# pairlab/SlotFormer

Measured on AMD Instinct MI355X. Metric: rollout frames/sec at B=32, 128x128, 7 slots, 6+50 steps (SAVi-encode + SlotFormer rollout), higher is better.
Workload: dtype f32 storage; matmul/conv on split-bf16 MFMA (bf16x3: hi*hi+hi*lo+lo*hi, f32 accumulate)

## Files before the change

slotformer_amd/csrc/layer_tok.hip:

```cpp
#include "../../include/slotformer_hip.h"
#include "sf_internal.h"
#include "layer_fused.h"
#include "layer_tok_common.h"
#include <stdlib.h>

namespace {
constexpr int LT_NT = 256, LT_D = 256, LT_F = 1024, LT_NH = 8, LT_TOK = 128, LT_MAXL = 8;
constexpr int LT_STAGE = 32 * 1024, LT_RING = 3;
constexpr int LT_NST_ATT = 4 * LT_NH, LT_NST = LT_NST_ATT + 2 * (LT_F / 32);
constexpr int LT_KV = LT_RING * LT_STAGE;
constexpr int LT_VT = LT_KV + 16 * 1024;
constexpr int LT_PAR = LT_KV + 32 * 1024;
constexpr int P_LN1G = 0, P_LN1B = 256, P_BQKV = 512, P_BO = 1280, P_LN2G = 1536, P_LN2B = 1792, P_B1 = 2048, P_B2 = 3072, P_N = 3328;
constexpr size_t LT_LDS = (size_t)LT_PAR + (size_t)P_N * 4;
constexpr size_t LT_BLOB = (size_t)LT_NST * LT_STAGE + (size_t)P_N * 4;
static_assert(LT_LDS <= 160 * 1024, "LDS budget");

struct LtArgs {
  const float* x;
  const float* ring;
  const float* pe;
  float* y;
  const char* blob[LT_MAXL];
  float eps;
  int nl, B, L, vpw, RF, N, f0, dbg_ts;
};
}

__device__ long long lt_ts[16];
#define LTS(i) do { if (A.dbg_ts && blockIdx.x == 0 && threadIdx.x == 0) lt_ts[i] = wall_clock64(); } while (0)

template <int MODE>
__global__ __launch_bounds__(LT_NT) void layer_tok_kernel(LtArgs A) {
  extern __shared__ __attribute__((aligned(16))) char smem[];
  float* P = (float*)(smem + LT_PAR);
  const int t = threadIdx.x, lane = t & 63;
  const int wave = __builtin_amdgcn_readfirstlane(t >> 6);
  const int n = lane & 31, h = lane >> 5;
  const int L = A.L;
  const int v0 = blockIdx.x * A.vpw;
  const int nvalid = min(A.vpw, A.B - v0) * L;
  const int tl = wave * 32 + n;
  const int te = min(tl, nvalid - 1);
  const int vl = te / L, tok = te - vl * L;
  const long long row = (long long)(v0 + vl) * L + tok;
  LTS(0);
  f32x16 X[8];
  if constexpr (MODE == 0) {
    const float* xr = A.x + row * LT_D + 4 * h;
#pragma unroll
    for (int ob = 0; ob < 8; ++ob)
#pragma unroll
      for (int g = 0; g < 4; ++g) {
        const f32x4 v = *(const f32x4*)(xr + 32 * ob + 8 * g);
#pragma unroll
        for (int q = 0; q < 4; ++q) X[ob][4 * g + q] = v[q];
      }
  } else {
    const int fr = tok / A.N, sl = tok - fr * A.N;
    const float* rr = A.ring + (((long long)(v0 + vl) * A.RF + (A.f0 + fr) % A.RF) * A.N + sl) * LT_D + 4 * h;
    const float* pr = A.pe + (long long)tok * LT_D + 4 * h;
#pragma unroll
    for (int ob = 0; ob < 8; ++ob)
#pragma unroll
      for (int g = 0; g < 4; ++g) {
        const f32x4 v = *(const f32x4*)(rr + 32 * ob + 8 * g);
#pragma unroll
        for (int q = 0; q < 4; ++q) X[ob][4 * g + q] = v[q];
      }
    __builtin_amdgcn_sched_barrier(0);
#pragma unroll
    for (int ob = 0; ob < 8; ++ob) {
#pragma unroll
      for (int g = 0; g < 4; ++g) {
        const f32x4 v = *(const f32x4*)(pr + 32 * ob + 8 * g);
#pragma unroll
        for (int q = 0; q < 4; ++q) X[ob][4 * g + q] += v[q];
      }
      __builtin_amdgcn_sched_barrier(0);
    }
  }
  const unsigned wlane = (unsigned)(wave * 8 * 1024 + lane * 16);
  char* const wdst = smem + (wave * 8) * 1024;
  int cur = 0;
  int cs = -2;
  const char* base_cur = A.blob[0];
  const char* base_nxt = A.blob[0];
  bool last_layer = false;
  auto stage_src = [&]() -> const char* {
    const int t2 = cs + 2;
    const bool wrap = t2 >= LT_NST;
    const char* b = wrap ? base_nxt : base_cur;
    const int so = wrap ? (last_layer ? LT_NST - 1 : t2 - LT_NST) : t2;
    ++cs;
    return b + (size_t)so * LT_STAGE + wlane;
  };
  {
    const char* s0 = stage_src();
    const char* s1 = stage_src();
    LtRing R0{nullptr, s0, wdst}, R1{nullptr, s1, wdst + LT_STAGE};
#pragma unroll
    for (int f = 0; f < 8; ++f) lt_dma(R0, f);
#pragma unroll
    for (int f = 0; f < 8; ++f) lt_dma(R1, f);
  }
#ifdef LT_STAMPS
  long long c_wait = 0, c_bar = 0, c_last = 0, c_work = 0;
#endif
  auto stage_begin = [&]() -> LtRing {
#ifdef LT_STAMPS
    const long long c0 = __builtin_readcyclecounter();
    if (c_last) c_work += c0 - c_last;
#endif
#ifdef LT_NODMA
    asm volatile("s_waitcnt vmcnt(0)" ::: "memory");
#else
    asm volatile("s_waitcnt vmcnt(8)" ::: "memory");
#endif
    asm volatile("s_waitcnt lgkmcnt(0)" ::: "memory");
#ifdef LT_STAMPS
    const long long c1 = __builtin_readcyclecounter();
#endif
#ifndef LT_NOBAR
    __builtin_amdgcn_s_barrier();
#endif
    asm volatile("" ::: "memory");
#ifdef LT_STAMPS
    c_last = __builtin_readcyclecounter();
    c_wait += c1 - c0;
    c_bar += c_last - c1;
#endif
    const int nb = cur == 0 ? 2 : cur - 1;
    LtRing R{smem + cur * LT_STAGE + lane * 16, stage_src(), wdst + nb * LT_STAGE};
#ifdef LT_BURST
#pragma unroll
    for (int f = 0; f < 8; ++f) lt_dma_now(R, f);
#endif
    cur = cur == 2 ? 0 : cur + 1;
    return R;
  };
  const int wf = min(wave * 32, nvalid - 1);
  const int kb0 = ((wf / L) * L) >> 5;
  const int d0 = 32 * kb0 + 4 * h - vl * L;
  const char* pb;
  {
    unsigned pbo = (unsigned)(LT_PAR + 16 * h);
    asm volatile("" : "+v"(pbo));
    pb = smem + pbo;
  }
  char* const kwr = smem + LT_KV + wave * 1024 + lane * 16;
  char* const vwr = smem + LT_VT + wave * 4096 + lane * 16;
  const char* krd[3];
  const char* vrd[3];
#pragma unroll
  for (int kbi = 0; kbi < 3; ++kbi) {
    const int kb = min(kb0 + kbi, 3);
    krd[kbi] = smem + LT_KV + kb * 1024 + lane * 16;
    vrd[kbi] = smem + LT_VT + kb * 4096 + lane * 16;
  }
  const float qscale = 0.2550348616841918f;
  constexpr float NEG = -3.0e38f;
  LTS(1);

#pragma unroll 1
  for (int l = 0; l < A.nl; ++l) {
    cs = 0;
    base_cur = A.blob[l];
    last_layer = l + 1 >= A.nl;
    base_nxt = A.blob[last_layer ? l : l + 1];
    __syncthreads();
    {
      const float* vsrc = (const float*)(A.blob[l] + (size_t)LT_NST * LT_STAGE);
      for (int i = t; i < P_N / 4; i += LT_NT) *(f32x4*)(P + 4 * i) = *(const f32x4*)(vsrc + 4 * i);
    }
    __syncthreads();
    if (l == 0) LTS(2);
    bf16x8 xh[16], xl[16];
    lt_layernorm<P_LN1G, P_LN1B>(X, pb, h, A.eps, xh, xl);
    lt_add_vec<P_BO>(X, pb);
    if (l == 0) LTS(3);
    f32x16 qa, ka, va, S[3], O;
    bf16x8 qh[2], ql[2], ph[3][2], pl[3][2], oh[2], ol[2];
    float mx0 = NEG, mx1 = NEG, mx = 0.f, sm = 0.f, rinv = 0.f;
    auto zero16 = [](f32x16& a) {
#pragma unroll
      for (int r = 0; r < 16; ++r) a[r] = 0.f;
    };
    int hq = 0;
    auto mask_chunk = [&](int c) {
      const int kbi = c >> 1;
#pragma unroll
      for (int rr = 0; rr < 8; ++rr) {
        const int r = 8 * (c & 1) + rr;
        const bool ok = (unsigned)(d0 + 32 * kbi + 8 * (r >> 2) + (r & 3)) < (unsigned)L;
        const float v = ok ? S[kbi][r] : NEG;
        S[kbi][r] = v;
        if (rr & 1) mx1 = fmaxf(mx1, v); else mx0 = fmaxf(mx0, v);
      }
    };
    auto exp_chunk = [&](int c) {
      const int kbi = c >> 1;
      float s0 = 0.f, s1 = 0.f;
#pragma unroll
      for (int rr = 0; rr < 8; ++rr) {
        const int r = 8 * (c & 1) + rr;
#ifdef LT_EXPF
        const float e = __expf((S[kbi][r] - mx) * 0.6931471805599453f);
#else
        const float e = __builtin_amdgcn_exp2f(S[kbi][r] - mx);
#endif
        S[kbi][r] = e;
        if (rr & 1) s1 += e; else s0 += e;
      }
      sm += s0 + s1;
    };
    auto psplit_chunk = [&](int c) { split8(quad(S[c >> 1], 2 * (c & 1)), quad(S[c >> 1], 2 * (c & 1) + 1), ph[c >> 1][c & 1], pl[c >> 1][c & 1]); };
    auto kconv = [&](int s) {
      const float* bk = (const float*)pb + P_BQKV + 256 + 32 * hq;
      bf16x8 fh, fl;
      split8(quad(ka, 2 * s) + *(const f32x4*)(bk + 16 * s), quad(ka, 2 * s + 1) + *(const f32x4*)(bk + 16 * s + 8), fh, fl);
      *(bf16x8*)(kwr + (s * 2) * 4096) = fh;
      *(bf16x8*)(kwr + (s * 2 + 1) * 4096) = fl;
    };
    auto qconv = [&](int s) {
      const float* bq = (const float*)pb + P_BQKV + 32 * hq;
      split8((quad(qa, 2 * s) + *(const f32x4*)(bq + 16 * s)) * qscale, (quad(qa, 2 * s + 1) + *(const f32x4*)(bq + 16 * s + 8)) * qscale, qh[s], ql[s]);
    };
    auto vconv = [&](int s) {
      const float bv = P[P_BQKV + 512 + 32 * hq + n];
      bf16x8 fh, fl;
      split8(quad(va, 2 * s) + bv, quad(va, 2 * s + 1) + bv, fh, fl);
      *(bf16x8*)(vwr + (s * 2) * 1024) = fh;
      *(bf16x8*)(vwr + (s * 2 + 1) * 1024) = fl;
    };
    auto oconv = [&](int s) { split8(quad(O, 2 * s) * rinv, quad(O, 2 * s + 1) * rinv, oh[s], ol[s]); };
    auto scores = [&]() {
      bf16x8 kh[3][2], kl[3][2];
#pragma unroll
      for (int kbi = 0; kbi < 3; ++kbi)
#pragma unroll
        for (int s = 0; s < 2; ++s) {
          kh[kbi][s] = *(const bf16x8*)(krd[kbi] + (s * 2) * 4096);
          kl[kbi][s] = *(const bf16x8*)(krd[kbi] + (s * 2 + 1) * 4096);
        }
#pragma unroll
      for (int kbi = 0; kbi < 3; ++kbi) zero16(S[kbi]);
#pragma unroll
      for (int s = 0; s < 2; ++s) {
#pragma unroll
        for (int kbi = 0; kbi < 3; ++kbi) { S[kbi] = LT_MFMA(kh[kbi][s], ql[s], S[kbi]); LT_PIN(); }
#pragma unroll
        for (int kbi = 0; kbi < 3; ++kbi) { S[kbi] = LT_MFMA(kl[kbi][s], qh[s], S[kbi]); LT_PIN(); }
#pragma unroll
        for (int kbi = 0; kbi < 3; ++kbi) { S[kbi] = LT_MFMA(kh[kbi][s], qh[s], S[kbi]); LT_PIN(); }
      }
      mx0 = mx1 = NEG;
      sm = 0.f;
    };
    auto pv = [&]() {
      f32x16 Op[3];
      bf16x8 vh[3][2], vlo[3][2];
#pragma unroll
      for (int kbi = 0; kbi < 3; ++kbi)
#pragma unroll
        for (int s = 0; s < 2; ++s) {
          vh[kbi][s] = *(const bf16x8*)(vrd[kbi] + (s * 2) * 1024);
          vlo[kbi][s] = *(const bf16x8*)(vrd[kbi] + (s * 2 + 1) * 1024);
        }
#pragma unroll
      for (int kbi = 0; kbi < 3; ++kbi) zero16(Op[kbi]);
#pragma unroll
      for (int s = 0; s < 2; ++s) {
#pragma unroll
        for (int kbi = 0; kbi < 3; ++kbi) { Op[kbi] = LT_MFMA(vh[kbi][s], pl[kbi][s], Op[kbi]); LT_PIN(); }
#pragma unroll
        for (int kbi = 0; kbi < 3; ++kbi) { Op[kbi] = LT_MFMA(vlo[kbi][s], ph[kbi][s], Op[kbi]); LT_PIN(); }
#pragma unroll
        for (int kbi = 0; kbi < 3; ++kbi) { Op[kbi] = LT_MFMA(vh[kbi][s], ph[kbi][s], Op[kbi]); LT_PIN(); }
      }
#pragma unroll
      for (int r = 0; r < 16; ++r) O[r] = (Op[0][r] + Op[1][r]) + Op[2][r];
    };
    auto sideD = [&](int g) {
      if (g < 6) mask_chunk(g);
      if (g == 6) mx = lt_xmax(fmaxf(mx0, mx1), h);
      if (g == 7) exp_chunk(0);
    };
    auto sideA = [&](int g) {
      if (g == 0) { exp_chunk(1); exp_chunk(2); }
      if (g == 1) { exp_chunk(3); exp_chunk(4); }
      if (g == 2) { exp_chunk(5); rinv = 1.0f / lt_xsum(sm, h); psplit_chunk(0); }
      if (g == 3) { psplit_chunk(1); psplit_chunk(2); }
      if (g == 4) { psplit_chunk(3); psplit_chunk(4); }
      if (g == 5) psplit_chunk(5);
    };
    {
      const LtRing R = stage_begin();
      lt_row_product<false, 0>(R, xh, xl, qa, LtNoSide{});
    }
    {
      const LtRing R = stage_begin();
      lt_row_product<false, 0>(R, xh, xl, ka, LtNoSide{});
    }
    {
      const LtRing R = stage_begin();
      lt_row_product<true, 5>(R, xh, xl, va, [&](int g) {
        if (g < 2) kconv(g);
        else if (g < 4) qconv(g - 2);
      });
      vconv(0);
      vconv(1);
    }
#pragma unroll 1
    for (hq = 1; hq < LT_NH; ++hq) {
      {
        const LtRing R = stage_begin();
        scores();
          lt_row_product<false, 6>(R, xh, xl, qa, sideD);
      }
      {
        const LtRing R = stage_begin();
          lt_row_product<false, 6>(R, xh, xl, ka, sideA);
        pv();
      }
      {
        const LtRing R = stage_begin();
          lt_row_product<true, 5>(R, xh, xl, va, [&](int g) {
          if (g < 2) kconv(g);
          else if (g < 4) qconv(g - 2);
          else if (g < 6) oconv(g - 4);
        });
      }
      {
        const LtRing R = stage_begin();
        lt_kslice_product<5>(R, oh, ol, X, [&](int g) {
          if (g < 2) vconv(g);
        });
      }
    }
    asm volatile("s_waitcnt lgkmcnt(0)" ::: "memory");
    __builtin_amdgcn_s_barrier();
    asm volatile("" ::: "memory");
    scores();
#pragma unroll
    for (int g = 0; g < 8; ++g) sideD(g);
#pragma unroll
    for (int g = 0; g < 6; ++g) sideA(g);
    pv();
    oconv(0);
    oconv(1);
    {
      const LtRing R = stage_begin();
      lt_kslice_product<0>(R, oh, ol, X, LtNoSide{});
    }
    if (l == 0) LTS(4);
#ifdef LT_STAMPS
    if (l == 0 && blockIdx.x == 0 && threadIdx.x == 0) { lt_ts[8] = c_wait; lt_ts[9] = c_bar; lt_ts[10] = c_work; }
#endif
    lt_layernorm<P_LN2G, P_LN2B>(X, pb, h, A.eps, xh, xl);
    lt_add_vec<P_B2>(X, pb);
    if (l == 0) LTS(5);
    f32x16 Ha, Hb;
    bf16x8 hh[2], hl[2];
    f32x4 b1q[4];
    auto b1_load = [&](int blk) {
      const float* b1 = (const float*)pb + P_B1 + 32 * blk;
#pragma unroll
      for (int g = 0; g < 4; ++g) b1q[g] = *(const f32x4*)(b1 + 8 * g);
    };
    auto hconv = [&](const f32x16& Hx, int s) {
      const f32x4 z4 = {0.f, 0.f, 0.f, 0.f};
      const f32x4 u0 = __builtin_elementwise_max(quad(Hx, 2 * s) + b1q[2 * s], z4);
      const f32x4 u1 = __builtin_elementwise_max(quad(Hx, 2 * s + 1) + b1q[2 * s + 1], z4);
      split8(u0, u1, hh[s], hl[s]);
    };
    auto ffn_step = [&](f32x16& Hn, const f32x16& Hp, int j) {
      {
        const LtRing R = stage_begin();
        lt_row_product<false, 4>(R, xh, xl, Hn, [&](int g) {
          if (g >= 1 && g < 3) hconv(Hp, g - 1);
        });
        asm volatile("" : "+v"(hh[0]), "+v"(hh[1]), "+v"(hl[0]), "+v"(hl[1]));
      }
      {
        const LtRing R = stage_begin();
        b1_load(j);
        lt_kslice_product<0>(R, hh, hl, X, LtNoSide{});
      }
    };
    {
      const LtRing R = stage_begin();
      b1_load(0);
      lt_row_product<false, 0>(R, xh, xl, Ha, LtNoSide{});
    }
    ffn_step(Hb, Ha, 1);
#pragma unroll 1
    for (int j = 2; j < LT_F / 32; j += 2) {
      ffn_step(Ha, Hb, j);
      ffn_step(Hb, Ha, j + 1);
    }
    hconv(Hb, 0);
    hconv(Hb, 1);
    {
      const LtRing R = stage_begin();
      lt_kslice_product<0>(R, hh, hl, X, LtNoSide{});
    }
    if (l == 0) LTS(6);
#ifdef LT_STAMPS
    if (l == 0 && blockIdx.x == 0 && threadIdx.x == 0) { lt_ts[11] = c_wait; lt_ts[12] = c_bar; lt_ts[13] = c_work; }
#endif
  }
  asm volatile("s_waitcnt vmcnt(0)" ::: "memory");
  if (tl < nvalid) {
    float* yr = A.y + row * LT_D + 4 * h;
#pragma unroll
    for (int ob = 0; ob < 8; ++ob)
#pragma unroll
      for (int g = 0; g < 4; ++g) *(f32x4*)(yr + 32 * ob + 8 * g) = quad(X[ob], g);
  }
  LTS(7);
}

extern "C" int sf_debug_read_ts_layer_tok(long long* out16) {
  hipError_t e = hipMemcpyFromSymbol(out16, HIP_SYMBOL(lt_ts), sizeof(long long) * 16);
  return e == hipSuccess ? 0 : (int)e;
}

extern "C" size_t sf_layer_tok_packed_bytes(void) { return LT_BLOB; }
extern "C" size_t sf_layer_tok_packed_bytes_ex(int d_model, int num_heads, int ffn) {
  if (d_model == LT_D && num_heads == LT_NH && ffn == LT_F) return LT_BLOB;
  return sf_layer_tok128_shape(d_model, num_heads, ffn) ? sf_layer_tok128_packed_bytes() : 0;
}

extern "C" int sf_pack_layer_tok_weights(const sf_tfm_layer* w, void* packed, int d_model, int num_heads, int ffn, void* stream) {
  SF_REQUIRE(w && packed, "sf_pack_layer_tok_weights: null pointer");
  SF_REQUIRE(w->in_proj_w && w->out_proj_w && w->lin1_w && w->lin2_w && w->norm1_g && w->norm1_b && w->in_proj_b && w->out_proj_b && w->norm2_g &&
                 w->norm2_b && w->lin1_b && w->lin2_b, "sf_pack_layer_tok_weights: null weight");
  hipStream_t st = (hipStream_t)stream;
  if (sf_layer_tok128_shape(d_model, num_heads, ffn)) return sf_pack_layer_tok128(w, packed, st);
  SF_REQUIRE(d_model == LT_D && num_heads == LT_NH && ffn == LT_F, "sf_pack_layer_tok_weights: (d_model, heads, ffn) = (256, 8, 1024) or (128, 8, 512) only");
  const int total = LT_NST * 32 * 64;
  hipLaunchKernelGGL((pack_layer_tok_kernel<LT_D, LT_F>), dim3((total + 255) / 256), dim3(256), 0, st, w->in_proj_w, w->out_proj_w, w->lin1_w, w->lin2_w, (uint4*)packed);
  SF_CHECK_LAUNCH();
  float* vec = (float*)((char*)packed + (size_t)LT_NST * LT_STAGE);
  const struct {
    const float* src;
    int off, n;
  } parts[8] = {{w->norm1_g, P_LN1G, 256}, {w->norm1_b, P_LN1B, 256}, {w->in_proj_b, P_BQKV, 768}, {w->out_proj_b, P_BO, 256},
                {w->norm2_g, P_LN2G, 256}, {w->norm2_b, P_LN2B, 256}, {w->lin1_b, P_B1, 1024},   {w->lin2_b, P_B2, 256}};
  for (const auto& p : parts) {
    const hipError_t e = hipMemcpyAsync(vec + p.off, p.src, (size_t)p.n * 4, hipMemcpyDeviceToDevice, st);
    if (e != hipSuccess) return sf_set_err((int)e, hipGetErrorString(e), __FILE__, __LINE__);
  }
  return 0;
}

int sf_layer_tok_vpw(int L) {
  if (L < 1 || L > 96) return 0;
  for (int vpw = LT_TOK / L; vpw >= 1; --vpw) {
    const int nvalid = vpw * L;
    bool ok = true;
    for (int w = 0; w < 4 && ok; ++w) {
      const int wf = w * 32 < nvalid ? w * 32 : nvalid - 1, wl = w * 32 + 31 < nvalid ? w * 32 + 31 : nvalid - 1;
      const int kb0 = ((wf / L) * L) >> 5, kb1 = (((wl / L) * L) + L - 1) >> 5;
      ok = kb1 - kb0 + 1 <= 3;
    }
    if (ok) return vpw;
  }
  return 0;
}
bool sf_layer_tok_ok(int L) { return sf_layer_tok_vpw(L) > 0; }

int sf_layer_tok_ex(int mode, const float* xin, const float* ring, int ring_frames, int nslots, int f0, const float* pe, const sf_tfm_layer* layers, int nl,
                    float eps, float* y, int B, int L, hipStream_t st) {
  bool ok = layers && nl >= 1 && nl <= LT_MAXL && sf_layer_tok_ok(L) && B >= 1 && y && (mode == 0 ? xin != nullptr : (ring && pe && nslots >= 1 && ring_frames >= 1));
  for (int l = 0; ok && l < nl; ++l) ok = layers[l].tok_packed != nullptr;
  if (!ok)
    return sf_set_err(-1, "invalid argument: the token-stationary layers need sf_pack_layer_tok_weights fragments, 1..8 layers and 1 <= L <= 96 rows per video", __FILE__, __LINE__);
  static const int dbg = sf_dbg("lt");
  LtArgs A;
  A.x = xin; A.ring = ring; A.pe = pe; A.y = y;
  for (int l = 0; l < LT_MAXL; ++l) A.blob[l] = (const char*)layers[l < nl ? l : nl - 1].tok_packed;
  A.eps = eps; A.nl = nl; A.B = B; A.L = L; A.vpw = sf_layer_tok_vpw(L); A.RF = ring_frames; A.N = nslots; A.f0 = f0; A.dbg_ts = dbg;
  const int nwg = (B + A.vpw - 1) / A.vpw;
  const double flops = nl * ((double)B * L * (2.0 * LT_D * (3 * LT_D + LT_D + 2 * LT_F)) + (double)B * LT_NH * 4.0 * L * L * 32);
  if (mode == 0) {
    SF_TRY(sf_ensure_dyn_lds((const void*)layer_tok_kernel<0>, LT_LDS));
    sf_prof_begin(SF_K_LAYER_TOK, st, flops);
    hipLaunchKernelGGL(layer_tok_kernel<0>, dim3(nwg), dim3(LT_NT), LT_LDS, st, A);
  } else {
    SF_TRY(sf_ensure_dyn_lds((const void*)layer_tok_kernel<1>, LT_LDS));
    sf_prof_begin(SF_K_LAYER_TOK, st, flops);
    hipLaunchKernelGGL(layer_tok_kernel<1>, dim3(nwg), dim3(LT_NT), LT_LDS, st, A);
  }
  sf_prof_end(SF_K_LAYER_TOK, st);
  SF_CHECK_LAUNCH();
  return 0;
}

extern "C" int sf_layer_tok_block_f32(const sf_tfm_layer* w, int nl, const float* x, float* y, int B, int L, void* stream) {
  SF_REQUIRE(w && x && y && B > 0 && nl >= 1 && nl <= LT_MAXL, "sf_layer_tok_block_f32: null pointer / empty problem / more than 8 layers");
  SF_REQUIRE(sf_get_precision() == 1, "sf_layer_tok_block_f32: split-bf16 mode only");
  return sf_layer_tok_ex(0, x, nullptr, 1, 1, 0, nullptr, w, nl, 1e-5f, y, B, L, (hipStream_t)stream);
}

extern "C" int sf_layer_tok_block_ex_f32(const sf_tfm_layer* w, int nl, int d_model, int num_heads, int ffn, const float* x, float* y, int B, int L,
                                         void* stream) {
  SF_REQUIRE(w && x && y && B > 0 && nl >= 1 && nl <= LT_MAXL, "sf_layer_tok_block_ex_f32: null pointer / empty problem / more than 8 layers");
  SF_REQUIRE(sf_get_precision() == 1, "sf_layer_tok_block_ex_f32: split-bf16 mode only");
  if (sf_layer_tok128_shape(d_model, num_heads, ffn)) return sf_layer_tok128_ex(x, w, nl, 1e-5f, y, B, L, (hipStream_t)stream);
  SF_REQUIRE(d_model == LT_D && num_heads == LT_NH && ffn == LT_F, "sf_layer_tok_block_ex_f32: (d_model, heads, ffn) = (256, 8, 1024) or (128, 8, 512) only");
  return sf_layer_tok_ex(0, x, nullptr, 1, 1, 0, nullptr, w, nl, 1e-5f, y, B, L, (hipStream_t)stream);
}
```

slotformer_amd/csrc/layer_tok_common.h:

```cpp
#pragma once
#include "../../include/slotformer_hip.h"
#include "sf_internal.h"

typedef float f32x16 __attribute__((ext_vector_type(16)));
typedef float f32x4 __attribute__((ext_vector_type(4)));
typedef __bf16 bf16x4 __attribute__((ext_vector_type(4)));
typedef __bf16 bf16x8 __attribute__((ext_vector_type(8)));

namespace {
__device__ __forceinline__ bf16x8 cat8(bf16x4 a, bf16x4 b) { return __builtin_shufflevector(a, b, 0, 1, 2, 3, 4, 5, 6, 7); }
__device__ __forceinline__ void split8(const f32x4 a, const f32x4 b, bf16x8& hi, bf16x8& lo) {
  const bf16x4 h0 = __builtin_convertvector(a, bf16x4), h1 = __builtin_convertvector(b, bf16x4);
  const bf16x4 l0 = __builtin_convertvector(a - __builtin_convertvector(h0, f32x4), bf16x4);
  const bf16x4 l1 = __builtin_convertvector(b - __builtin_convertvector(h1, f32x4), bf16x4);
  hi = cat8(h0, h1);
  lo = cat8(l0, l1);
}
__device__ __forceinline__ f32x4 quad(const f32x16& a, int g) { return f32x4{a[4 * g], a[4 * g + 1], a[4 * g + 2], a[4 * g + 3]}; }
__device__ __forceinline__ float lt_xother(float v, int h) {
#ifdef LT_SHFL
  return __shfl_xor(v, 32, 64);
#endif
  const unsigned u = __builtin_bit_cast(unsigned, v);
  const auto r = __builtin_amdgcn_permlane32_swap(u, u, false, false);
  return __builtin_bit_cast(float, h ? r[0] : r[1]);
}
__device__ __forceinline__ float lt_xmax(float v, int h) { return fmaxf(v, lt_xother(v, h)); }
__device__ __forceinline__ float lt_xsum(float v, int h) {
  const float o = lt_xother(v, h);
  return h ? o + v : v + o;
}

struct LtRing {
  const char* rd;
  const char* src;
  char* dst;
};
__device__ __forceinline__ void lt_dma_now(const LtRing& R, int f) {
  __builtin_amdgcn_global_load_lds((const void __attribute__((address_space(1)))*)(R.src + f * 1024),
                                   (void __attribute__((address_space(3)))*)(R.dst + f * 1024), 16, 0, 0);
}
__device__ __forceinline__ void lt_dma(const LtRing& R, int f) {
#if defined(LT_NODMA) || defined(LT_BURST)
  return;
#endif
#ifndef LT_NOIMMOFF
  const void __attribute__((address_space(1)))* s = (const void __attribute__((address_space(1)))*)(R.src + (f >> 2) * 4096);
  void __attribute__((address_space(3)))* d = (void __attribute__((address_space(3)))*)(R.dst + (f >> 2) * 4096);
  switch (f & 3) {
    case 0: __builtin_amdgcn_global_load_lds(s, d, 16, 0, 0); break;
    case 1: __builtin_amdgcn_global_load_lds(s, d, 16, 1024, 0); break;
    case 2: __builtin_amdgcn_global_load_lds(s, d, 16, 2048, 0); break;
    default: __builtin_amdgcn_global_load_lds(s, d, 16, 3072, 0); break;
  }
#else
  __builtin_amdgcn_global_load_lds((const void __attribute__((address_space(1)))*)(R.src + f * 1024),
                                   (void __attribute__((address_space(3)))*)(R.dst + f * 1024), 16, 0, 0);
#endif
}
#define LT_MFMA(a, b, c) __builtin_amdgcn_mfma_f32_32x32x16_bf16(a, b, c, 0, 0, 0)
#define LT_PIN() __builtin_amdgcn_sched_barrier(0x7F6)
#define LT_SGB(mask, n) __builtin_amdgcn_sched_group_barrier(mask, n, 0)
struct LtNoSide {
  __device__ __forceinline__ void operator()(int) const {}
};
template <int NV, bool READS>
__device__ __forceinline__ void lt_group_pattern() {
  LT_SGB(0x008, 1);
  if constexpr (READS) LT_SGB(0x100, 4);
#pragma unroll
  for (int k = 0; k < 5; ++k) {
    if constexpr (NV > 0) LT_SGB(0x002, NV);
    LT_SGB(0x008, 1);
  }
  if constexpr (NV > 0) LT_SGB(0x002, NV);
  __builtin_amdgcn_sched_barrier(0);
}

template <bool SW, int NV, int NKS, class Side>
__device__ __forceinline__ void lt_row_product(const LtRing& R, const bf16x8 (&xh)[NKS], const bf16x8 (&xl)[NKS], f32x16& a, Side&& side) {
  constexpr int NG = NKS / 2;
  bf16x8 wb[2][4];
  f32x16 a1;
#pragma unroll
  for (int r = 0; r < 16; ++r) a[r] = a1[r] = 0.f;
#pragma unroll
  for (int i = 0; i < 4; ++i) wb[0][i] = *(const bf16x8*)(R.rd + i * 1024);
#pragma unroll
  for (int g = 0; g < NG; ++g) {
    const int b = g & 1, ks = 2 * g;
    if constexpr (!SW) a = LT_MFMA(wb[b][0], xl[ks], a); else a = LT_MFMA(xl[ks], wb[b][0], a);
#ifndef LT_NOREAD
    if (g + 1 < NG) {
#pragma unroll
      for (int i = 0; i < 4; ++i) wb[b ^ 1][i] = *(const bf16x8*)(R.rd + (4 * (g + 1) + i) * 1024);
    }
#else
    if (g == 0) {
#pragma unroll
      for (int i = 0; i < 4; ++i) wb[1][i] = *(const bf16x8*)(R.rd + (4 + i) * 1024);
    }
#endif
    lt_dma(R, g);
    LT_PIN();
    if constexpr (!SW) {
      a1 = LT_MFMA(wb[b][2], xl[ks + 1], a1);
      LT_PIN();
      a = LT_MFMA(wb[b][1], xh[ks], a);
      LT_PIN();
      a1 = LT_MFMA(wb[b][3], xh[ks + 1], a1);
      LT_PIN();
      a = LT_MFMA(wb[b][0], xh[ks], a);
      LT_PIN();
      a1 = LT_MFMA(wb[b][2], xh[ks + 1], a1);
    } else {
      a1 = LT_MFMA(xl[ks + 1], wb[b][2], a1);
      LT_PIN();
      a = LT_MFMA(xh[ks], wb[b][1], a);
      LT_PIN();
      a1 = LT_MFMA(xh[ks + 1], wb[b][3], a1);
      LT_PIN();
      a = LT_MFMA(xh[ks], wb[b][0], a);
      LT_PIN();
      a1 = LT_MFMA(xh[ks + 1], wb[b][2], a1);
    }
    LT_PIN();
#ifndef LT_NOSIDE
    side(g);
    if (g + 1 < NG) lt_group_pattern<NV, true>(); else lt_group_pattern<NV, false>();
#else
    if (g + 1 < NG) lt_group_pattern<0, true>(); else lt_group_pattern<0, false>();
#endif
  }
#ifdef LT_NOSIDE
#pragma unroll
  for (int g = 0; g < NG; ++g) side(g);
#endif
#pragma unroll
  for (int r = 0; r < 16; ++r) a[r] += a1[r];
}
template <int NV, int NOB, class Side>
__device__ __forceinline__ void lt_kslice_product(const LtRing& R, const bf16x8 (&ih)[2], const bf16x8 (&il)[2], f32x16 (&Y)[NOB], Side&& side) {
  bf16x8 wb[2][8];
#pragma unroll
  for (int i = 0; i < 8; ++i) wb[0][i] = *(const bf16x8*)(R.rd + i * 1024);
#pragma unroll
  for (int p = 0; p < NOB / 2; ++p) {
    const int b = p & 1, oa = 2 * p, ob = 2 * p + 1;
    Y[oa] = LT_MFMA(wb[b][0], il[0], Y[oa]);
#ifndef LT_NOREAD
    if (p + 1 < NOB / 2) {
#pragma unroll
      for (int i = 0; i < 8; ++i) wb[b ^ 1][i] = *(const bf16x8*)(R.rd + (8 * (p + 1) + i) * 1024);
    }
#else
    if (p == 0) {
#pragma unroll
      for (int i = 0; i < 8; ++i) wb[1][i] = *(const bf16x8*)(R.rd + (8 + i) * 1024);
    }
#endif
    lt_dma(R, 2 * p);
    LT_PIN();
    Y[ob] = LT_MFMA(wb[b][4], il[0], Y[ob]);
    LT_PIN();
    Y[oa] = LT_MFMA(wb[b][1], ih[0], Y[oa]);
    LT_PIN();
    Y[ob] = LT_MFMA(wb[b][5], ih[0], Y[ob]);
    LT_PIN();
    Y[oa] = LT_MFMA(wb[b][0], ih[0], Y[oa]);
    LT_PIN();
    Y[ob] = LT_MFMA(wb[b][4], ih[0], Y[ob]);
    lt_dma(R, 2 * p + 1);
    LT_PIN();
    Y[oa] = LT_MFMA(wb[b][2], il[1], Y[oa]);
    LT_PIN();
    Y[ob] = LT_MFMA(wb[b][6], il[1], Y[ob]);
    LT_PIN();
    Y[oa] = LT_MFMA(wb[b][3], ih[1], Y[oa]);
    LT_PIN();
    Y[ob] = LT_MFMA(wb[b][7], ih[1], Y[ob]);
    LT_PIN();
    Y[oa] = LT_MFMA(wb[b][2], ih[1], Y[oa]);
    LT_PIN();
    Y[ob] = LT_MFMA(wb[b][6], ih[1], Y[ob]);
    LT_PIN();
#ifndef LT_NOSIDE
    side(2 * p);
    side(2 * p + 1);
#endif
    LT_SGB(0x008, 1);
    if (p + 1 < NOB / 2) LT_SGB(0x100, 8);
#pragma unroll
    for (int k = 0; k < 11; ++k) {
      if constexpr (NV > 0) LT_SGB(0x002, NV);
      LT_SGB(0x008, 1);
    }
    if constexpr (NV > 0) LT_SGB(0x002, NV);
    __builtin_amdgcn_sched_barrier(0);
  }
#ifdef LT_NOSIDE
#pragma unroll
  for (int g = 0; g < NOB; ++g) side(g);
#endif
}

template <int GOFF, int BOFF, int NOB>
__device__ __forceinline__ void lt_layernorm(const f32x16 (&X)[NOB], const char* pb, int h, float eps, bf16x8 (&xh)[2 * NOB], bf16x8 (&xl)[2 * NOB]) {
  float s0 = 0.f, s1 = 0.f, s2 = 0.f, s3 = 0.f;
#pragma unroll
  for (int ob = 0; ob < NOB; ++ob)
#pragma unroll
    for (int r = 0; r < 16; r += 4) {
      s0 += X[ob][r];
      s1 += X[ob][r + 1];
      s2 += X[ob][r + 2];
      s3 += X[ob][r + 3];
    }
  const float mu = lt_xsum((s0 + s1) + (s2 + s3), h) * (1.0f / (32 * NOB));
  float q0 = 0.f, q1 = 0.f, q2 = 0.f, q3 = 0.f;
#pragma unroll
  for (int ob = 0; ob < NOB; ++ob)
#pragma unroll
    for (int r = 0; r < 16; r += 4) {
      const float d0 = X[ob][r] - mu, d1 = X[ob][r + 1] - mu, d2 = X[ob][r + 2] - mu, d3 = X[ob][r + 3] - mu;
      q0 += d0 * d0;
      q1 += d1 * d1;
      q2 += d2 * d2;
      q3 += d3 * d3;
    }
  const float rs = 1.0f / sqrtf(lt_xsum((q0 + q1) + (q2 + q3), h) * (1.0f / (32 * NOB)) + eps);
#pragma unroll
  for (int ob = 0; ob < NOB; ++ob)
#pragma unroll
    for (int s2i = 0; s2i < 2; ++s2i) {
      f32x4 v[2];
#pragma unroll
      for (int gg = 0; gg < 2; ++gg) {
        const int g = 2 * s2i + gg, c = 32 * ob + 8 * g;
        v[gg] = (quad(X[ob], g) - mu) * rs * *(const f32x4*)(pb + (GOFF + c) * 4) + *(const f32x4*)(pb + (BOFF + c) * 4);
      }
      split8(v[0], v[1], xh[2 * ob + s2i], xl[2 * ob + s2i]);
      __builtin_amdgcn_sched_barrier(0);
    }
}
template <int OFF, int NOB>
__device__ __forceinline__ void lt_add_vec(f32x16 (&X)[NOB], const char* pb) {
#pragma unroll
  for (int ob = 0; ob < NOB; ++ob) {
#pragma unroll
    for (int g = 0; g < 4; ++g) {
      const f32x4 bv = *(const f32x4*)(pb + (OFF + 32 * ob + 8 * g) * 4);
#pragma unroll
      for (int q = 0; q < 4; ++q) X[ob][4 * g + q] += bv[q];
    }
    __builtin_amdgcn_sched_barrier(0);
  }
}

template <int D, int F>
__global__ void pack_layer_tok_kernel(const float* __restrict__ win, const float* __restrict__ wout, const float* __restrict__ w1,
                                      const float* __restrict__ w2, uint4* __restrict__ out) {
  constexpr int NB = D / 32, FPS = D / 8, NST_ATT = 4 * NB, NFF = 2 * (F / 32), NST = NST_ATT + NFF;
  const int idx = blockIdx.x * blockDim.x + threadIdx.x;
  if (idx >= NST * FPS * 64) return;
  const int lane = idx & 63, f = (idx >> 6) % FPS, st = idx / (64 * FPS);
  const int pl = f & 1, h = lane >> 5, i = lane & 31;
  const float* W;
  int ld, r0 = 0, c0 = 0, s;
  bool slice;
  if (st < NST_ATT) {
    int hd, kind;
    if (st < 3) {
      hd = 0; kind = st;
    } else if (st == NST_ATT - 1) {
      hd = NB - 1; kind = 3;
    } else {
      const int tq = st - 3;
      kind = tq & 3;
      hd = 1 + (tq >> 2) - (kind == 3 ? 1 : 0);
    }
    slice = kind == 3;
    ld = D;
    if (!slice) {
      W = win; r0 = kind * D + 32 * hd;
    } else {
      W = wout; c0 = 32 * hd;
    }
  } else {
    const int ff = st - NST_ATT;
    int hb;
    if (ff == 0) {
      slice = false; hb = 0;
    } else if (ff == NFF - 1) {
      slice = true; hb = F / 32 - 1;
    } else if (ff & 1) {
      slice = false; hb = (ff + 1) >> 1;
    } else {
      slice = true; hb = (ff >> 1) - 1;
    }
    if (!slice) {
      W = w1; ld = D; r0 = 32 * hb;
    } else {
      W = w2; ld = F; c0 = 32 * hb;
    }
  }
  if (!slice) {
    const int vk = f >> 1;
    c0 = 32 * (vk >> 1);
    s = vk & 1;
  } else {
    r0 = 32 * (f >> 2);
    s = (f >> 1) & 1;
  }
  const float* src = W + (long long)(r0 + i) * ld + c0 + 4 * h;
  union {
    __bf16 b[8];
    uint4 u;
  } o;
#pragma unroll
  for (int j = 0; j < 8; ++j) {
    const float v = src[8 * (2 * s + (j >> 2)) + (j & 3)];
    const __bf16 hi = (__bf16)v;
    o.b[j] = pl ? (__bf16)(v - (float)hi) : hi;
  }
  out[idx] = o.u;
}
}
```

Baseline: 661,300.

## Rebalance attention side work across MFMA groups with finer-grained bf16 splits

Replaces the 8-wide bf16 hi/lo split with 2- and 4-element packed splits so that mask, exp, split, and Q/K/V/O conversion work can be spread evenly across the eight MFMA groups of each row product. K conversion moves after the PV MFMAs, O is reduced and split incrementally during the V product, and V conversion moves into the output k-slice product. Scheduling patterns gain a transcendental group slot and a new run pattern. The intent is to hide VALU and transcendental latency behind MFMAs in the per-head attention pipeline, at the cost of more live registers and more complex scheduling hints.

```diff
diff --git a/slotformer_amd/csrc/layer_tok.hip b/slotformer_amd/csrc/layer_tok.hip
--- a/slotformer_amd/csrc/layer_tok.hip
+++ b/slotformer_amd/csrc/layer_tok.hip
@@ -179,61 +179,71 @@
     lt_layernorm<P_LN1G, P_LN1B>(X, pb, h, A.eps, xh, xl);
     lt_add_vec<P_BO>(X, pb);
     if (l == 0) LTS(3);
-    f32x16 qa, ka, va, S[3], O;
-    bf16x8 qh[2], ql[2], ph[3][2], pl[3][2], oh[2], ol[2];
-    float mx0 = NEG, mx1 = NEG, mx = 0.f, sm = 0.f, rinv = 0.f;
+    f32x16 qa, ka, va, S[3], Op[3];
+    bf16x8 qh[2], ql[2], oh[2], ol[2];
+    u32x4 phu[3][2], plu[3][2], qhu[2], qlu[2], ohu[2], olu[2], kfh, kfl, vfh, vfl;
+    float mx0 = NEG, mx1 = NEG, mx = 0.f, sm = 0.f, es0 = 0.f, es1 = 0.f, rinv = 0.f, bv = 0.f;
     auto zero16 = [](f32x16& a) {
 #pragma unroll
       for (int r = 0; r < 16; ++r) a[r] = 0.f;
     };
     int hq = 0;
-    auto mask_chunk = [&](int c) {
-      const int kbi = c >> 1;
-#pragma unroll
-      for (int rr = 0; rr < 8; ++rr) {
-        const int r = 8 * (c & 1) + rr;
+    auto mask12 = [&](int c) {
+#pragma unroll
+      for (int f = 12 * c; f < 12 * c + 12; ++f) {
+        const int kbi = f >> 4, r = f & 15;
         const bool ok = (unsigned)(d0 + 32 * kbi + 8 * (r >> 2) + (r & 3)) < (unsigned)L;
         const float v = ok ? S[kbi][r] : NEG;
         S[kbi][r] = v;
-        if (rr & 1) mx1 = fmaxf(mx1, v); else mx0 = fmaxf(mx0, v);
-      }
-    };
-    auto exp_chunk = [&](int c) {
-      const int kbi = c >> 1;
-      float s0 = 0.f, s1 = 0.f;
-#pragma unroll
-      for (int rr = 0; rr < 8; ++rr) {
-        const int r = 8 * (c & 1) + rr;
+        if (r & 1) mx1 = fmaxf(mx1, v); else mx0 = fmaxf(mx0, v);
+      }
+    };
+    auto exp4 = [&](int k) {
+      const int kbi = k >> 2, r0 = 4 * (k & 3);
+      if (!(k & 1)) es0 = es1 = 0.f;
+#pragma unroll
+      for (int rr = 0; rr < 4; ++rr) {
 #ifdef LT_EXPF
-        const float e = __expf((S[kbi][r] - mx) * 0.6931471805599453f);
+        const float e = __expf((S[kbi][r0 + rr] - mx) * 0.6931471805599453f);
 #else
-        const float e = __builtin_amdgcn_exp2f(S[kbi][r] - mx);
-#endif
-        S[kbi][r] = e;
-        if (rr & 1) s1 += e; else s0 += e;
-      }
-      sm += s0 + s1;
-    };
-    auto psplit_chunk = [&](int c) { split8(quad(S[c >> 1], 2 * (c & 1)), quad(S[c >> 1], 2 * (c & 1) + 1), ph[c >> 1][c & 1], pl[c >> 1][c & 1]); };
-    auto kconv = [&](int s) {
+        const float e = __builtin_amdgcn_exp2f(S[kbi][r0 + rr] - mx);
+#endif
+        S[kbi][r0 + rr] = e;
+        if (rr & 1) es1 += e; else es0 += e;
+      }
+      if (k & 1) sm += es0 + es1;
+      split4(quad(S[kbi], k & 3), phu[kbi][(k >> 1) & 1], plu[kbi][(k >> 1) & 1], k & 1);
+    };
+    auto kconv4 = [&](int j) {
       const float* bk = (const float*)pb + P_BQKV + 256 + 32 * hq;
-      bf16x8 fh, fl;
-      split8(quad(ka, 2 * s) + *(const f32x4*)(bk + 16 * s), quad(ka, 2 * s + 1) + *(const f32x4*)(bk + 16 * s + 8), fh, fl);
-      *(bf16x8*)(kwr + (s * 2) * 4096) = fh;
-      *(bf16x8*)(kwr + (s * 2 + 1) * 4096) = fl;
-    };
-    auto qconv = [&](int s) {
+      split4(quad(ka, j) + *(const f32x4*)(bk + 8 * j), kfh, kfl, j & 1);
+      if (j & 1) {
+        *(u32x4*)(kwr + ((j >> 1) * 2) * 4096) = kfh;
+        *(u32x4*)(kwr + ((j >> 1) * 2 + 1) * 4096) = kfl;
+      }
+    };
+    auto qconv4 = [&](int j) {
       const float* bq = (const float*)pb + P_BQKV + 32 * hq;
-      split8((quad(qa, 2 * s) + *(const f32x4*)(bq + 16 * s)) * qscale, (quad(qa, 2 * s + 1) + *(const f32x4*)(bq + 16 * s + 8)) * qscale, qh[s], ql[s]);
-    };
-    auto vconv = [&](int s) {
-      const float bv = P[P_BQKV + 512 + 32 * hq + n];
-      bf16x8 fh, fl;
-      split8(quad(va, 2 * s) + bv, quad(va, 2 * s + 1) + bv, fh, fl);
-      *(bf16x8*)(vwr + (s * 2) * 1024) = fh;
-      *(bf16x8*)(vwr + (s * 2 + 1) * 1024) = fl;
-    };
-    auto oconv = [&](int s) { split8(quad(O, 2 * s) * rinv, quad(O, 2 * s + 1) * rinv, oh[s], ol[s]); };
+      split4((quad(qa, j) + *(const f32x4*)(bq + 8 * j)) * qscale, qhu[j >> 1], qlu[j >> 1], j & 1);
+      if (j & 1) { qh[j >> 1] = lt_frag(qhu[j >> 1]); ql[j >> 1] = lt_frag(qlu[j >> 1]); }
+    };
+    auto vconv4 = [&](int j) {
+      if (j == 0) bv = P[P_BQKV + 512 + 32 * hq + n];
+      split4(quad(va, j) + bv, vfh, vfl, j & 1);
+      if (j & 1) {
+        *(u32x4*)(vwr + ((j >> 1) * 2) * 1024) = vfh;
+        *(u32x4*)(vwr + ((j >> 1) * 2 + 1) * 1024) = vfl;
+      }
+    };
+    auto oconv2 = [&](int g) {
+      if (g == 0) rinv = 1.0f / lt_xsum(sm, h);
+      const float o0 = ((Op[0][2 * g] + Op[1][2 * g]) + Op[2][2 * g]) * rinv, o1 = ((Op[0][2 * g + 1] + Op[1][2 * g + 1]) + Op[2][2 * g + 1]) * rinv;
+      unsigned hw, lw;
+      split2(o0, o1, hw, lw);
+      ohu[g >> 2][g & 3] = hw;
+      olu[g >> 2][g & 3] = lw;
+      if ((g & 3) == 3) { oh[g >> 2] = lt_frag(ohu[g >> 2]); ol[g >> 2] = lt_frag(olu[g >> 2]); }
+    };
     auto scores = [&]() {
       bf16x8 kh[3][2], kl[3][2];
 #pragma unroll
@@ -257,8 +267,7 @@
       mx0 = mx1 = NEG;
       sm = 0.f;
     };
-    auto pv = [&]() {
-      f32x16 Op[3];
+    auto pv = [&](auto withk) {
       bf16x8 vh[3][2], vlo[3][2];
 #pragma unroll
       for (int kbi = 0; kbi < 3; ++kbi)
@@ -272,27 +281,29 @@
 #pragma unroll
       for (int s = 0; s < 2; ++s) {
 #pragma unroll
-        for (int kbi = 0; kbi < 3; ++kbi) { Op[kbi] = LT_MFMA(vh[kbi][s], pl[kbi][s], Op[kbi]); LT_PIN(); }
-#pragma unroll
-        for (int kbi = 0; kbi < 3; ++kbi) { Op[kbi] = LT_MFMA(vlo[kbi][s], ph[kbi][s], Op[kbi]); LT_PIN(); }
-#pragma unroll
-        for (int kbi = 0; kbi < 3; ++kbi) { Op[kbi] = LT_MFMA(vh[kbi][s], ph[kbi][s], Op[kbi]); LT_PIN(); }
-      }
-#pragma unroll
-      for (int r = 0; r < 16; ++r) O[r] = (Op[0][r] + Op[1][r]) + Op[2][r];
+        for (int kbi = 0; kbi < 3; ++kbi) { Op[kbi] = LT_MFMA(vh[kbi][s], lt_frag(plu[kbi][s]), Op[kbi]); LT_PIN(); }
+#pragma unroll
+        for (int kbi = 0; kbi < 3; ++kbi) { Op[kbi] = LT_MFMA(vlo[kbi][s], lt_frag(phu[kbi][s]), Op[kbi]); LT_PIN(); }
+#pragma unroll
+        for (int kbi = 0; kbi < 3; ++kbi) { Op[kbi] = LT_MFMA(vh[kbi][s], lt_frag(phu[kbi][s]), Op[kbi]); LT_PIN(); }
+      }
+      if constexpr (decltype(withk)::value) {
+#pragma unroll
+        for (int j = 0; j < 4; ++j) kconv4(j);
+#ifndef LT_NOSIDE
+        lt_run_pattern<5, 18>();
+#endif
+      }
     };
     auto sideD = [&](int g) {
-      if (g < 6) mask_chunk(g);
-      if (g == 6) mx = lt_xmax(fmaxf(mx0, mx1), h);
-      if (g == 7) exp_chunk(0);
-    };
-    auto sideA = [&](int g) {
-      if (g == 0) { exp_chunk(1); exp_chunk(2); }
-      if (g == 1) { exp_chunk(3); exp_chunk(4); }
-      if (g == 2) { exp_chunk(5); rinv = 1.0f / lt_xsum(sm, h); psplit_chunk(0); }
-      if (g == 3) { psplit_chunk(1); psplit_chunk(2); }
-      if (g == 4) { psplit_chunk(3); psplit_chunk(4); }
-      if (g == 5) psplit_chunk(5);
+      if (g < 4) mask12(g);
+      if (g == 4) mx = lt_xmax(fmaxf(mx0, mx1), h);
+      if (g >= 4) exp4(g - 4);
+    };
+    auto sideA = [&](int g) { exp4(g + 4); };
+    auto sideB = [&](int g) { oconv2(g); };
+    auto sideC = [&](int g) {
+      if (g & 1) qconv4(g >> 1); else vconv4(g >> 1);
     };
     {
       const LtRing R = stage_begin();
@@ -305,37 +316,31 @@
     {
       const LtRing R = stage_begin();
       lt_row_product<true, 5>(R, xh, xl, va, [&](int g) {
-        if (g < 2) kconv(g);
-        else if (g < 4) qconv(g - 2);
+        if (g < 4) kconv4(g);
+        else qconv4(g - 4);
       });
-      vconv(0);
-      vconv(1);
+#pragma unroll
+      for (int j = 0; j < 4; ++j) vconv4(j);
     }
 #pragma unroll 1
     for (hq = 1; hq < LT_NH; ++hq) {
       {
         const LtRing R = stage_begin();
         scores();
-          lt_row_product<false, 6>(R, xh, xl, qa, sideD);
+        lt_row_product<false, 5, 1>(R, xh, xl, qa, sideD);
       }
       {
         const LtRing R = stage_begin();
-          lt_row_product<false, 6>(R, xh, xl, ka, sideA);
-        pv();
+        lt_row_product<false, 4, 1>(R, xh, xl, ka, sideA);
+        pv(LtYes{});
       }
       {
         const LtRing R = stage_begin();
-          lt_row_product<true, 5>(R, xh, xl, va, [&](int g) {
-          if (g < 2) kconv(g);
-          else if (g < 4) qconv(g - 2);
-          else if (g < 6) oconv(g - 4);
-        });
+        lt_row_product<true, 6, 1>(R, xh, xl, va, sideB);
       }
       {
         const LtRing R = stage_begin();
-        lt_kslice_product<5>(R, oh, ol, X, [&](int g) {
-          if (g < 2) vconv(g);
-        });
+        lt_kslice_product<5>(R, oh, ol, X, sideC);
       }
     }
     asm volatile("s_waitcnt lgkmcnt(0)" ::: "memory");
@@ -345,10 +350,10 @@
 #pragma unroll
     for (int g = 0; g < 8; ++g) sideD(g);
 #pragma unroll
-    for (int g = 0; g < 6; ++g) sideA(g);
-    pv();
-    oconv(0);
-    oconv(1);
+    for (int g = 0; g < 8; ++g) sideA(g);
+    pv(LtNo{});
+#pragma unroll
+    for (int g = 0; g < 8; ++g) sideB(g);
     {
       const LtRing R = stage_begin();
       lt_kslice_product<0>(R, oh, ol, X, LtNoSide{});
@@ -362,25 +367,25 @@
     if (l == 0) LTS(5);
     f32x16 Ha, Hb;
     bf16x8 hh[2], hl[2];
+    u32x4 hhu[2], hlu[2];
     f32x4 b1q[4];
     auto b1_load = [&](int blk) {
       const float* b1 = (const float*)pb + P_B1 + 32 * blk;
 #pragma unroll
       for (int g = 0; g < 4; ++g) b1q[g] = *(const f32x4*)(b1 + 8 * g);
     };
-    auto hconv = [&](const f32x16& Hx, int s) {
+    auto hconv4 = [&](const f32x16& Hx, int j) {
       const f32x4 z4 = {0.f, 0.f, 0.f, 0.f};
-      const f32x4 u0 = __builtin_elementwise_max(quad(Hx, 2 * s) + b1q[2 * s], z4);
-      const f32x4 u1 = __builtin_elementwise_max(quad(Hx, 2 * s + 1) + b1q[2 * s + 1], z4);
-      split8(u0, u1, hh[s], hl[s]);
+      split4(__builtin_elementwise_max(quad(Hx, j) + b1q[j], z4), hhu[j >> 1], hlu[j >> 1], j & 1);
     };
     auto ffn_step = [&](f32x16& Hn, const f32x16& Hp, int j) {
       {
         const LtRing R = stage_begin();
         lt_row_product<false, 4>(R, xh, xl, Hn, [&](int g) {
-          if (g >= 1 && g < 3) hconv(Hp, g - 1);
+          if (g >= 1 && g < 5) hconv4(Hp, g - 1);
         });
-        asm volatile("" : "+v"(hh[0]), "+v"(hh[1]), "+v"(hl[0]), "+v"(hl[1]));
+        asm volatile("" : "+v"(hhu[0]), "+v"(hhu[1]), "+v"(hlu[0]), "+v"(hlu[1]));
+        hh[0] = lt_frag(hhu[0]); hh[1] = lt_frag(hhu[1]); hl[0] = lt_frag(hlu[0]); hl[1] = lt_frag(hlu[1]);
       }
       {
         const LtRing R = stage_begin();
@@ -399,8 +404,9 @@
       ffn_step(Ha, Hb, j);
       ffn_step(Hb, Ha, j + 1);
     }
-    hconv(Hb, 0);
-    hconv(Hb, 1);
+#pragma unroll
+    for (int j = 0; j < 4; ++j) hconv4(Hb, j);
+    hh[0] = lt_frag(hhu[0]); hh[1] = lt_frag(hhu[1]); hl[0] = lt_frag(hlu[0]); hl[1] = lt_frag(hlu[1]);
     {
       const LtRing R = stage_begin();
       lt_kslice_product<0>(R, hh, hl, X, LtNoSide{});
diff --git a/slotformer_amd/csrc/layer_tok_common.h b/slotformer_amd/csrc/layer_tok_common.h
--- a/slotformer_amd/csrc/layer_tok_common.h
+++ b/slotformer_amd/csrc/layer_tok_common.h
@@ -9,12 +9,41 @@
 
 namespace {
 __device__ __forceinline__ bf16x8 cat8(bf16x4 a, bf16x4 b) { return __builtin_shufflevector(a, b, 0, 1, 2, 3, 4, 5, 6, 7); }
+typedef float f32x2 __attribute__((ext_vector_type(2)));
+typedef __bf16 bf16x2 __attribute__((ext_vector_type(2)));
+typedef unsigned u32x4 __attribute__((ext_vector_type(4)));
+__device__ __forceinline__ void split2(float a, float b, unsigned& hi, unsigned& lo) {
+#ifndef LT_PKSPLIT
+  const __bf16 h0 = (__bf16)a, h1 = (__bf16)b;
+  const bf16x2 hv = {h0, h1}, lv = {(__bf16)(a - (float)h0), (__bf16)(b - (float)h1)};
+  hi = __builtin_bit_cast(unsigned, hv);
+  lo = __builtin_bit_cast(unsigned, lv);
+#else
+  const unsigned p = __builtin_bit_cast(unsigned, __builtin_convertvector((f32x2{a, b}), bf16x2));
+  const float ha = __builtin_bit_cast(float, p << 16), hb = __builtin_bit_cast(float, p & 0xffff0000u);
+#ifdef LT_PKSUB
+  const f32x2 r = f32x2{a, b} - f32x2{ha, hb};
+#else
+  const f32x2 r = {a - ha, b - hb};
+#endif
+  hi = p;
+  lo = __builtin_bit_cast(unsigned, __builtin_convertvector(r, bf16x2));
+#endif
+}
+__device__ __forceinline__ void split4(const f32x4 a, u32x4& hi, u32x4& lo, int half) {
+  unsigned h0, l0, h1, l1;
+  split2(a[0], a[1], h0, l0);
+  split2(a[2], a[3], h1, l1);
+  hi[2 * half] = h0; hi[2 * half + 1] = h1;
+  lo[2 * half] = l0; lo[2 * half + 1] = l1;
+}
+__device__ __forceinline__ bf16x8 lt_frag(const u32x4 v) { return __builtin_bit_cast(bf16x8, v); }
 __device__ __forceinline__ void split8(const f32x4 a, const f32x4 b, bf16x8& hi, bf16x8& lo) {
-  const bf16x4 h0 = __builtin_convertvector(a, bf16x4), h1 = __builtin_convertvector(b, bf16x4);
-  const bf16x4 l0 = __builtin_convertvector(a - __builtin_convertvector(h0, f32x4), bf16x4);
-  const bf16x4 l1 = __builtin_convertvector(b - __builtin_convertvector(h1, f32x4), bf16x4);
-  hi = cat8(h0, h1);
-  lo = cat8(l0, l1);
+  u32x4 h, l;
+  split4(a, h, l, 0);
+  split4(b, h, l, 1);
+  hi = lt_frag(h);
+  lo = lt_frag(l);
 }
 __device__ __forceinline__ f32x4 quad(const f32x16& a, int g) { return f32x4{a[4 * g], a[4 * g + 1], a[4 * g + 2], a[4 * g + 3]}; }
 __device__ __forceinline__ float lt_xother(float v, int h) {
@@ -61,23 +90,40 @@
 #define LT_MFMA(a, b, c) __builtin_amdgcn_mfma_f32_32x32x16_bf16(a, b, c, 0, 0, 0)
 #define LT_PIN() __builtin_amdgcn_sched_barrier(0x7F6)
 #define LT_SGB(mask, n) __builtin_amdgcn_sched_group_barrier(mask, n, 0)
+struct LtYes {
+  static constexpr bool value = true;
+};
+struct LtNo {
+  static constexpr bool value = false;
+};
 struct LtNoSide {
   __device__ __forceinline__ void operator()(int) const {}
 };
-template <int NV, bool READS>
+template <int NV, bool READS, int NT = 0>
 __device__ __forceinline__ void lt_group_pattern() {
   LT_SGB(0x008, 1);
   if constexpr (READS) LT_SGB(0x100, 4);
 #pragma unroll
   for (int k = 0; k < 5; ++k) {
     if constexpr (NV > 0) LT_SGB(0x002, NV);
+    if constexpr (NT > 0) LT_SGB(0x400, NT);
     LT_SGB(0x008, 1);
   }
   if constexpr (NV > 0) LT_SGB(0x002, NV);
+  if constexpr (NT > 0) LT_SGB(0x400, NT);
   __builtin_amdgcn_sched_barrier(0);
 }
-
-template <bool SW, int NV, int NKS, class Side>
+template <int NV, int N>
+__device__ __forceinline__ void lt_run_pattern() {
+#pragma unroll
+  for (int k = 0; k < N; ++k) {
+    LT_SGB(0x008, 1);
+    if constexpr (NV > 0) LT_SGB(0x002, NV);
+  }
+  __builtin_amdgcn_sched_barrier(0);
+}
+
+template <bool SW, int NV, int NT = 0, int NKS, class Side>
 __device__ __forceinline__ void lt_row_product(const LtRing& R, const bf16x8 (&xh)[NKS], const bf16x8 (&xl)[NKS], f32x16& a, Side&& side) {
   constexpr int NG = NKS / 2;
   bf16x8 wb[2][4];
@@ -127,7 +173,7 @@
     LT_PIN();
 #ifndef LT_NOSIDE
     side(g);
-    if (g + 1 < NG) lt_group_pattern<NV, true>(); else lt_group_pattern<NV, false>();
+    if (g + 1 < NG) lt_group_pattern<NV, true, NT>(); else lt_group_pattern<NV, false, NT>();
 #else
     if (g + 1 < NG) lt_group_pattern<0, true>(); else lt_group_pattern<0, false>();
 #endif
```

Measured after the change: 654,600 (median of 2 runs). 1.0% lower.
